# accre/lstore

Hardware: AMD Instinct MI355X
Metric: erasure encode+decode GiB/s (device-resident), RS(6+3) 1 MiB stripes (higher is better)
Workload: dtype u8; 1 GPU; reed_sol_van(6+3) encode + decode(lost shard 0), C=1048576 B per shard, 4096 stripes/GPU, k*C=6291456 B user data per stripe; method=reed_sol_van, k=6, m=3, chunk_bytes=1048576, packet_size=4096, stripes_per_gpu=4096, parallelism=static stripe partition x1

## Files before the change

### lstore_amd/csrc/ec_kernels.h

```cpp
#pragma once

#include <hip/hip_runtime.h>
#include <stdint.h>

#include <tuple>
#include <utility>

namespace lsec {

template <typename T, size_t... I>
hipError_t launch_packed(const void *k, dim3 grid, dim3 block, hipStream_t st, T &args, std::index_sequence<I...>) {
  void *ptrs[] = {static_cast<void *>(&std::get<I>(args))..., nullptr};
  return hipLaunchKernel(k, grid, block, ptrs, 0, st);
}
template <typename... KArgs, typename... Args>
hipError_t launch_kernel(void (*k)(KArgs...), dim3 grid, dim3 block, hipStream_t st, const Args &...args) {
  static_assert(sizeof...(KArgs) == sizeof...(Args), "argument count");
  std::tuple<std::decay_t<KArgs>...> t(static_cast<std::decay_t<KArgs>>(args)...);
  return launch_packed(reinterpret_cast<const void *>(k), grid, block, st, t, std::index_sequence_for<KArgs...>{});
}

size_t occupancy_lds_bytes(int64_t shard_bytes);
template <typename T, size_t... I>
hipError_t launch_packed_shm(const void *k, dim3 grid, dim3 block, size_t shm, hipStream_t st, T &args,
// ... 66 lines not shown
struct PatternArgs {
  const PatRecord *recs;
  const CoefCell *cells;
  const uint8_t *stripe_pattern;
  uint32_t npat;
  uint32_t rot0, rot_step, rot_n;
  int K;
  int nstripes;
  int packet;
  int nshards;
  int64_t size;
  unsigned *tiles;
  uint32_t tiles_pre;
  uint32_t tile_phase;
  ShardRef sh[kPatMaxShards];
};

hipError_t launch_pattern_bytewise(const PatternArgs &a, int rmax, hipStream_t stream);
hipError_t launch_pattern_bitsliced(const PatternArgs &a, int rmax, hipStream_t stream);

struct CheckArgs {
  const CoefCell *cells;
  int K, R;
  int nstripes;
  int packet;
  int64_t size;
  unsigned *syndrome;
  unsigned *bad_count;
  unsigned *tiles;
  uint32_t tiles_pre;
  uint32_t tile_phase;
  ShardRef in[kMaxK];
  ShardRef par[kMaxR];
};

hipError_t launch_check_bytewise(const CheckArgs &a, hipStream_t stream);
hipError_t launch_check_bitsliced(const CheckArgs &a, hipStream_t stream, int dw_pref = 0);

struct LocateArgs : CheckArgs {
  const CoefCell *ratio;
  unsigned long long *hyp;
};

constexpr unsigned kLocateClean = 0xFF, kLocateMany = 0xFE;

hipError_t launch_locate_bytewise(const LocateArgs &a, hipStream_t stream);
hipError_t launch_locate_bitsliced(const LocateArgs &a, hipStream_t stream, int dw_pref = 0);
hipError_t launch_locate_finalize(const unsigned *syndrome, unsigned long long *hyp, unsigned char *located,
                                  unsigned *counts, int nstripes, int K, int R, hipStream_t stream);

constexpr int kRotMaxShards = kMaxK + 8;
struct CheckRotArgs {
  const CoefCell *cells;
  int K, R;
  int nstripes;
  int packet;
  int64_t size;
  unsigned *syndrome;
  unsigned *bad_count;
  unsigned *tiles;
  uint32_t tiles_pre;
  uint32_t tile_phase;
  uint32_t rot0, rot_step, rot_n;
  ShardRef sh[kRotMaxShards];
};

struct LocateRotArgs : CheckRotArgs {
  const CoefCell *ratio;
  unsigned long long *hyp;
};

hipError_t launch_check_rot_bytewise(const CheckRotArgs &a, hipStream_t stream);
hipError_t launch_check_rot_bitsliced(const CheckRotArgs &a, hipStream_t stream, int dw_pref = 0);
hipError_t launch_locate_rot_bytewise(const LocateRotArgs &a, hipStream_t stream);
hipError_t launch_locate_rot_bitsliced(const LocateRotArgs &a, hipStream_t stream, int dw_pref = 0);
hipError_t launch_locate_finalize_rot(const unsigned *syndrome, unsigned long long *hyp, unsigned char *located,
                                      unsigned char *located_dev, unsigned *counts, unsigned *dev_faults, int nstripes,
                                      int K, int R, uint32_t rot0, uint32_t rot_step, uint32_t rot_n, hipStream_t stream);

struct PatternRotArgs : PatternArgs {};
hipError_t launch_pattern_rot_bytewise(const PatternRotArgs &a, hipStream_t stream);
hipError_t launch_pattern_rot_bitsliced(const PatternRotArgs &a, hipStream_t stream);

enum LaunchFamily { kFormChk = 1, kFormLoc, kFormChkRot, kFormLocRot, kFormPat, kFormPatRot };
struct LaunchForm {
  int family, sliced, R, KC, IT, VW, BF, DW;
};
constexpr int kLaunchRecordMax = 16;
void record_launch(const LaunchForm &f);
void launch_record_reset();
int launch_record(LaunchForm *out, int max);
bool predict_launch(int family, bool sliced, int K, int R, int packet, int dw_pref, LaunchForm *out);
int fixed_k_list(int *out, int max);

constexpr int kTileQueueLine = 32;
constexpr int kTileQueueWords = 9 * kTileQueueLine;
constexpr int kTileQueueRing = 4096;
constexpr uint64_t kTileQueueMinTiles = 16384;
unsigned *tile_queue_slot(hipStream_t st, uint64_t ntiles);
bool tile_phase_on();
bool tile_phase_net_on();
void set_tile_phase(int mode);
void tile_queue_release(hipStream_t st, unsigned *slot);
uint32_t tiles_prefix(uint32_t ntiles);
unsigned long long *launch_stamps(uint32_t *n);
void set_launch_stamps(unsigned long long *p, uint32_t n);
int persistent_grid(const void *kernel, int grid, hipStream_t st);

constexpr int kMaxMagicShards = kMaxK + kMaxR;

struct MagicArgs {
  int nshards;
  int shard0;
  int total_shards;
  int nstripes;
  int64_t size;
  int64_t col0;
  int64_t chunk;
  unsigned long long *acc;
  ShardRef sh[kMaxMagicShards];
};

hipError_t launch_stripe_magic(const MagicArgs &a, hipStream_t stream);
hipError_t launch_magic_finalize(const unsigned long long *acc, int nstripes, int64_t total_len, uint8_t *magic,
                                 hipStream_t stream);

struct DiffArgs {
  int npairs;
  int nstripes;
  int64_t size;
  int *flags;
  ShardRef a[kMaxR];
  ShardRef b[kMaxR];
};
hipError_t launch_chunk_diff(const DiffArgs &a, hipStream_t stream);

struct GatherPiece {
  uint64_t src;
  uint64_t dst_off;
  uint64_t bytes;
};
hipError_t launch_gather(const GatherPiece *list, int n, char *dst, hipStream_t stream);

constexpr uint32_t kPieceBytes = 16384;
struct CopyPiece {
  uint64_t src;
  uint64_t dst;
  uint64_t bytes;
};
hipError_t launch_copy_pieces(const CopyPiece *list, int n, hipStream_t stream);

hipError_t launch_signal(unsigned *counter, unsigned *flag, unsigned value, hipStream_t stream);

hipError_t launch_hbm_copy(void *dst, const void *src, uint64_t bytes, hipStream_t stream);
hipError_t launch_hbm_mix(const ApplyArgs &a, hipStream_t stream);
hipError_t launch_probe_xor(const ShardRef *in, int K, ShardRef out, int nstripes, int64_t size, int variant,
                            hipStream_t stream);

void make_cell(uint8_t c, CoefCell &cell);

hipError_t launch_bytewise(const ApplyArgs &a, hipStream_t stream, int grid_blocks = 0);
hipError_t launch_bytewise_magic(const ApplyArgs &a, hipStream_t stream, int grid_blocks = 0);
hipError_t launch_bitsliced(const ApplyArgs &a, hipStream_t stream, int grid_blocks = 0, int dw_pref = 0);
hipError_t launch_bitmatrix(const ApplyArgs &a, hipStream_t stream, int grid_blocks = 0);
bool bitmatrix_w_supported(int w);
hipError_t launch_wordwise(const ApplyArgs &a, hipStream_t stream, int grid_blocks = 0);
hipError_t launch_gfw_bitsliced(const ApplyArgs &a, hipStream_t stream, int grid_blocks = 0);
void make_word_cell(uint32_t c, int w, uint32_t *out);

void set_kernel_variant(int bytewise_variant, int bitsliced_variant);
void set_tile_mode(int mode);
int tile_mode();
int bytewise_variant();
int bitsliced_variant();

}
```

### lstore_amd/csrc/ec_kernels.hip

```cpp
#include <atomic>
#include <cstdio>
#include <cstdlib>
#include <cstring>
#include <map>
#include <mutex>
#include <type_traits>

#include "ec_hiperr.h"
#include "ec_kernels_impl.h"

namespace lsec {

namespace {

int g_bw_variant = 0, g_bs_variant = 0;

int default_grid(uint64_t ntiles) {
  return static_cast<int>(std::min<uint64_t>(std::max<uint64_t>(ntiles, 1), (1ull << 31) - 1));
}

constexpr int kQueueDevs = 64;
std::once_flag g_queue_once[kQueueDevs];
unsigned *g_queue[kQueueDevs];
std::atomic<uint32_t> g_queue_next[kQueueDevs];
// ... 152 lines not shown
int tile_phase_mode() {
  int v = g_tile_phase.load(std::memory_order_relaxed);
  if (v < 0) {
    const char *e = getenv("LSEC_TILE_PHASE");
    v = e && *e ? (atoi(e) & 3) : 1;
    int expect = -1;
    if (!g_tile_phase.compare_exchange_strong(expect, v)) v = expect;
  }
  return v;
}
}

bool tile_phase_on() { return (tile_phase_mode() & 1) != 0; }
bool tile_phase_net_on() { return (tile_phase_mode() & 2) != 0; }

void set_tile_phase(int mode) { g_tile_phase.store(mode & 3, std::memory_order_relaxed); }

size_t occupancy_lds_bytes(int64_t shard_bytes) {
  static const int cap = [] {
    const char *e = getenv("LSEC_WGS_CAP");
    return e ? std::max(0, atoi(e)) : 0;
  }();
  static const int64_t min_bytes = [] {
    const char *e = getenv("LSEC_WGS_CAP_MIN_KB");
    return e ? static_cast<int64_t>(atoll(e)) << 10 : 0;
  }();
  if (cap <= 0 || shard_bytes < min_bytes) return 0;
  const size_t per = (160u << 10) / static_cast<size_t>(cap);
  return per > (2u << 10) ? (per - (2u << 10)) & ~static_cast<size_t>(255) : 0;
}

int persistent_grid(const void *kernel, int grid, hipStream_t st) {
  const int dev = stream_device(st);
  if (dev < 0 || dev >= kQueueDevs || g_cus[dev] <= 0) return 0;
  static std::mutex mu;
  static std::map<const void *, int> per_cu;
  int n = 0;
  {
    std::lock_guard<std::mutex> lk(mu);
    auto it = per_cu.find(kernel);
    if (it != per_cu.end()) {
      n = it->second;
    } else {
      if (quiet([&] { return hipOccupancyMaxActiveBlocksPerMultiprocessor(&n, kernel, kBlock, 0); }) != hipSuccess) n = 0;
      per_cu[kernel] = n;
    }
  }
  static const int force = [] {
    const char *e = getenv("LSEC_TILES_WGS");
    return e ? atoi(e) : 0;
  }();
  if (force > 0) n = force;
  static const int cap = [] {
    const char *e = getenv("LSEC_WGS_CAP");
    return e ? std::max(0, atoi(e)) : 0;
  }();
  if (cap > 0 && n > cap) n = cap;
  if (n <= 0) return 0;
  const int full = n * g_cus[dev];
  const int pg = std::max(8, std::min(grid, full) & ~7);
  static const bool trace = getenv("LSEC_TRACE") != nullptr;
  if (trace) fprintf(stderr, "[lsec tiles] kernel %p: %d workgroups per CU x %d CUs -> grid %d (of %d tiles)\n", kernel, n, g_cus[dev], pg, grid);
  return pg;
}

void set_tile_mode(int mode) { g_tiles_mode.store(std::max(0, std::min(2, mode)), std::memory_order_relaxed); }

int tile_mode() { return tiles_mode(); }

uint32_t tiles_prefix(uint32_t ntiles) {
  if (tiles_mode() != 2) return 0;
  const uint64_t per = (static_cast<uint64_t>(ntiles) + 7) / 8;
  return static_cast<uint32_t>(per * prefix_64ths() / 64);
}

void set_kernel_variant(int bw, int bs) {
  g_bw_variant = bw;
  g_bs_variant = bs;
}

int bytewise_variant() { return g_bw_variant; }
int bitsliced_variant() { return g_bs_variant; }

hipError_t launch_bytewise(const ApplyArgs &a, hipStream_t st, int grid_blocks) {
  if (a.K < 1 || a.K > kMaxK || a.R < 1 || a.R > 8 || a.size % 8 != 0) return hipErrorInvalidValue;
  if (a.nstripes <= 0 || a.size == 0) return hipSuccess;
  const int shape = a.accumulate ? 1 : bytewise_shape(a.K, a.R);
  const int grid = tile_grid(bw_shape(shape).tile_bytes(), a.size, a.nstripes, grid_blocks);
  if (!grid) return hipErrorInvalidValue;
  return by_r(a.R, [&](auto r) { return dispatch_bytewise<decltype(r)::value>(a, st, grid, shape); });
}

hipError_t launch_bytewise_magic(const ApplyArgs &a, hipStream_t st, int grid_blocks) {
  if (a.K < 1 || a.K > kMaxK || a.R < 1 || a.R > 8 || a.size % 8 != 0 || !a.magic_acc) return hipErrorInvalidValue;
  if (a.nstripes <= 0 || a.size == 0) return hipSuccess;
  const int grid = tile_grid(BwShape{bytewise_magic_it(a.K), 4, true}.tile_bytes(), a.size, a.nstripes, grid_blocks);
  if (!grid) return hipErrorInvalidValue;
  return by_r(a.R, [&](auto r) { return dispatch_bytewise_magic<decltype(r)::value>(a, st, grid); });
}

hipError_t launch_bitsliced(const ApplyArgs &a, hipStream_t st, int grid_blocks, int dw_pref) {
  if (a.K < 1 || a.K > kMaxK || a.R < 1 || a.R > 8 || a.packet <= 0 || a.packet % 4 != 0 ||
      a.size % (8LL * a.packet) != 0)
    return hipErrorInvalidValue;
  if (a.nstripes <= 0 || a.size == 0) return hipSuccess;
  const int want = g_bs_variant != 0 ? g_bs_variant : dw_pref;
  const int dw = lane_dwords(!a.magic_acc && !a.accumulate ? want : 1, a.packet);
  const int grid = tile_grid(kBlock * 4ull * dw, a.size / 8, a.nstripes, grid_blocks);
  if (!grid) return hipErrorInvalidValue;
  return by_r(a.R, [&](auto r) { return dispatch_bitsliced<decltype(r)::value>(a, st, grid, dw); });
}

bool bitmatrix_w_supported(int w) {
  switch (w) {
#define LSEC_BM_CASE(WW) case WW:
    LSEC_BITMATRIX_W(LSEC_BM_CASE)
#undef LSEC_BM_CASE
    return true;
    default:
      return false;
  }
}

hipError_t launch_bitmatrix(const ApplyArgs &a, hipStream_t st, int grid_blocks) {
  if (a.K < 1 || a.K > kMaxK || a.R < 1 || a.R > 2 || a.w < 2 || a.w > kMaxW || !a.masks ||
      a.packet <= 0 || a.packet % 4 != 0 || a.size % (static_cast<int64_t>(a.w) * a.packet) != 0)
    return hipErrorInvalidValue;
  if (a.nstripes <= 0 || a.size == 0) return hipSuccess;
  const int grid = tile_grid(kBlock * 4, a.size / a.w, a.nstripes, grid_blocks);
  if (!grid) return hipErrorInvalidValue;
  return by_r(a.R, [&](auto r) { return dispatch_bitmatrix<decltype(r)::value>(a, st, grid); });
}

hipError_t launch_wordwise(const ApplyArgs &a, hipStream_t st, int grid_blocks) {
  if (a.K < 1 || a.K > kMaxK || a.R < 1 || a.R > 8 || (a.w != 16 && a.w != 32) || !a.masks || a.size % 8 != 0)
    return hipErrorInvalidValue;
  if (a.nstripes <= 0 || a.size == 0) return hipSuccess;
  const bool transposed = g_bs_variant != 10 && (a.w == 16 || a.R <= 4);
  const int grid = tile_grid(kBlock * (transposed ? 4ull * a.w : a.w == 16 ? 16ull : 8ull), a.size, a.nstripes, grid_blocks);
  if (!grid) return hipErrorInvalidValue;
  if (transposed) return by_r(a.R, [&](auto r) { return dispatch_gfw_transposed<decltype(r)::value>(a, st, grid); });
  return by_r(a.R, [&](auto r) { return dispatch_wordwise<decltype(r)::value>(a, st, grid); });
}

hipError_t launch_gfw_bitsliced(const ApplyArgs &a, hipStream_t st, int grid_blocks) {
  if (a.K < 1 || a.K > kMaxK || a.R < 1 || a.R > (a.w == 32 ? 4 : 8) || (a.w != 16 && a.w != 32) || !a.masks ||
      a.packet <= 0 || a.packet % 4 != 0 || a.size % (static_cast<int64_t>(a.w) * a.packet) != 0)
    return hipErrorInvalidValue;
  if (a.nstripes <= 0 || a.size == 0) return hipSuccess;
  const int grid = tile_grid(kBlock * 4, a.size / a.w, a.nstripes, grid_blocks);
  if (!grid) return hipErrorInvalidValue;
  return by_r(a.R, [&](auto r) { return dispatch_gfw_bitsliced<decltype(r)::value>(a, st, grid); });
}

namespace {
bool pattern_args_ok(const PatternArgs &a, int rmax) {
  return a.K >= 1 && a.K <= kMaxK && rmax >= 1 && rmax <= kPatMaxOut && a.recs && a.cells && a.npat >= 1 &&
         a.npat <= kPatMaxPatterns && a.nshards >= 1 && a.nshards <= kPatMaxShards && a.size % 8 == 0 &&
         (a.stripe_pattern || (a.rot_n >= 1 && a.rot0 < a.rot_n && a.rot_step < a.rot_n && a.rot_n <= a.npat));
}
}

hipError_t launch_pattern_bytewise(const PatternArgs &a, int rmax, hipStream_t st) {
  if (!pattern_args_ok(a, rmax)) return hipErrorInvalidValue;
  if (a.nstripes <= 0 || a.size == 0) return hipSuccess;
  const int grid = tile_grid(bw_auto(a.K, rmax).tile_bytes(), a.size, a.nstripes);
  if (!grid) return hipErrorInvalidValue;
  return by_r(rmax, [&](auto r) { return dispatch_pat_bytewise<decltype(r)::value>(a, st, grid); });
}
// ... 581 lines not shown
```

### lstore_amd/csrc/ec_kernels_impl.h

```cpp
#pragma once
#include "ec_kernels.h"

#include <algorithm>
#include <type_traits>

namespace lsec {

typedef uint32_t u32x2 __attribute__((ext_vector_type(2)));
typedef uint32_t u32x4 __attribute__((ext_vector_type(4)));

template <int N> struct VecT;
template <> struct VecT<1> { typedef uint32_t type; };
template <> struct VecT<2> { typedef u32x2 type; };
template <> struct VecT<4> { typedef u32x4 type; };

constexpr int kBlock = 256;

typedef const __attribute__((address_space(4))) CoefCell ConstCell;

__device__ __forceinline__ ConstCell *const_cells(const CoefCell *p) {
  return reinterpret_cast<ConstCell *>(reinterpret_cast<uintptr_t>(p));
}

#define LSEC_GLOBAL __attribute__((address_space(1)))
// ... 966 lines not shown
          put<ACC, u32x2>(q0 + o, h);
        }
      }
    }
  }
}

template <int R, int W, bool ACC = false>
__global__ __launch_bounds__(kBlock) void k_gfw_transposed(ApplyArgs a) {
  constexpr uint32_t kCoefMask = W == 16 ? 0xFFFFu : 0xFFFFFFFFu;
  ConstU32 *prod = reinterpret_cast<ConstU32 *>(reinterpret_cast<uintptr_t>(a.masks));
  bool xor_only = true;
  for (int i = 0; i < R * a.K && xor_only; ++i) xor_only = (prod[i * W] & kCoefMask) <= 1u;
  if (xor_only)
    gfw_transposed_tiles<R, W, true, ACC>(a);
  else
    gfw_transposed_tiles<R, W, false, ACC>(a);
}

#define LSEC_BITMATRIX_W(X) X(2) X(3) X(4) X(5) X(6) X(7) X(8) X(10) X(11) X(12) X(13) X(16) X(17) \
                            X(18) X(19) X(22) X(23) X(28) X(29) X(30) X(31) X(32)

#define LSEC_FIXED_K(X) X(4) X(6) X(8) X(10) X(12) X(16) X(20)
constexpr bool has_fixed_k(int K) {
#define LSEC_IS_K(KK) \
  if (K == KK) return true;
  LSEC_FIXED_K(LSEC_IS_K)
#undef LSEC_IS_K
  return false;
}

struct BwShape {
  int it, vw;
  bool bf;
  constexpr uint64_t tile_bytes() const { return static_cast<uint64_t>(kBlock) * 4 * vw * it; }
};
constexpr int kBwShapes = 5;
constexpr BwShape bw_shape(int code) {
  return code == 0 ? BwShape{2, 4, true} : code == 1 ? BwShape{1, 4, true} : code == 2 ? BwShape{2, 2, true}
       : code == 3 ? BwShape{1, 2, true} : BwShape{1, 2, false};
}
constexpr int bw_auto_code(int K, int R) { return R == 1 ? 4 : K >= 16 ? 1 : 0; }
constexpr BwShape bw_auto(int K, int R) { return bw_shape(bw_auto_code(K, R)); }
constexpr int bytewise_magic_it(int K) { return bw_auto(K, 2).it; }

template <int R, int IT, bool BF, int VW>
hipError_t bytewise_k(const ApplyArgs &a, hipStream_t st, int grid) {
  switch (a.K) {
#define LSEC_BW_K(KK) \
  case KK: return launch_tiled(&k_gf8_bytewise<R, KK, IT, BF, VW>, grid, st, a);
    LSEC_FIXED_K(LSEC_BW_K)
#undef LSEC_BW_K
    default: return launch_tiled(&k_gf8_bytewise<R, 0, IT, BF, VW>, grid, st, a);
  }
}

template <int R>
hipError_t dispatch_bytewise(const ApplyArgs &a, hipStream_t st, int grid, int shape) {
  if (a.accumulate) {
    return launch_tiled(&k_gf8_bytewise<R, 0, 1, true, 4, false, true>, grid, st, a);
  }
  switch (shape) {
    case 1: return bytewise_k<R, 1, true, 4>(a, st, grid);
    case 2: return bytewise_k<R, 2, true, 2>(a, st, grid);
    case 3: return bytewise_k<R, 1, true, 2>(a, st, grid);
    case 4: return bytewise_k<R, 1, false, 2>(a, st, grid);
    default: return bytewise_k<R, 2, true, 4>(a, st, grid);
  }
}

template <int R>
hipError_t dispatch_bytewise_magic(const ApplyArgs &a, hipStream_t st, int grid) {
  switch (a.K) {
#define LSEC_BWM_K(KK) \
  case KK: return launch_tiled(&k_gf8_bytewise<R, KK, bytewise_magic_it(KK), true, 4, true>, grid, st, a);
    LSEC_FIXED_K(LSEC_BWM_K)
#undef LSEC_BWM_K
    default:
      if (bytewise_magic_it(a.K) == 1) return launch_tiled(&k_gf8_bytewise<R, 0, 1, true, 4, true>, grid, st, a);
      return launch_tiled(&k_gf8_bytewise<R, 0, 2, true, 4, true>, grid, st, a);
  }
}

template <int R>
hipError_t dispatch_bitsliced(const ApplyArgs &a, hipStream_t st, int grid, int dw) {
  if (a.magic_acc) {
    return launch_tiled(&k_gf8_bitsliced<R, 0, 1, true>, grid, st, a);
  }
  if (a.accumulate) {
    return launch_tiled(&k_gf8_bitsliced<R, 0, 1, false, true>, grid, st, a);
  }
  switch (dw) {
    case 4: return launch_tiled(&k_gf8_bitsliced<R, 0, 4>, grid, st, a);
    case 2: return launch_tiled(&k_gf8_bitsliced<R, 0, 2>, grid, st, a);
    default: return launch_tiled(&k_gf8_bitsliced<R, 0, 1>, grid, st, a);
  }
}

template <int R>
hipError_t dispatch_bitmatrix(const ApplyArgs &a, hipStream_t st, int grid) {
  if constexpr (R <= 2) {
    if (a.accumulate) {
      return launch_kernel(&k_bitmatrix_any<R>, dim3(grid), dim3(kBlock), st, a);
    }
    switch (a.w) {
#define LSEC_BM_W(WW) \
  case WW: return launch_kernel(&k_bitmatrix<R, WW>, dim3(grid), dim3(kBlock), st, a);
      LSEC_BITMATRIX_W(LSEC_BM_W)
#undef LSEC_BM_W
      default: return launch_kernel(&k_bitmatrix_any<R>, dim3(grid), dim3(kBlock), st, a);
    }
  } else {
    return hipErrorInvalidValue;
  }
}

template <int R>
hipError_t dispatch_wordwise(const ApplyArgs &a, hipStream_t st, int grid) {
  switch (a.w * 2 + (a.accumulate ? 1 : 0)) {
    case 32: return launch_kernel(&k_gfw_wordwise<R, 16>, dim3(grid), dim3(kBlock), st, a);
    case 33: return launch_kernel(&k_gfw_wordwise<R, 16, true>, dim3(grid), dim3(kBlock), st, a);
    case 64: return launch_kernel(&k_gfw_wordwise<R, 32>, dim3(grid), dim3(kBlock), st, a);
    case 65: return launch_kernel(&k_gfw_wordwise<R, 32, true>, dim3(grid), dim3(kBlock), st, a);
    default: return hipErrorInvalidValue;
  }
}

template <int R>
hipError_t dispatch_gfw_transposed(const ApplyArgs &a, hipStream_t st, int grid) {
  if (a.w == 16) {
    if (a.accumulate) return launch_kernel(&k_gfw_transposed<R, 16, true>, dim3(grid), dim3(kBlock), st, a);
    else return launch_kernel(&k_gfw_transposed<R, 16>, dim3(grid), dim3(kBlock), st, a);
  } else if constexpr (R <= 4) {
    if (a.w != 32) return hipErrorInvalidValue;
    if (a.accumulate) return launch_kernel(&k_gfw_transposed<R, 32, true>, dim3(grid), dim3(kBlock), st, a);
    else return launch_kernel(&k_gfw_transposed<R, 32>, dim3(grid), dim3(kBlock), st, a);
  } else {
    return hipErrorInvalidValue;
  }
}

template <int R>
hipError_t dispatch_gfw_bitsliced(const ApplyArgs &a, hipStream_t st, int grid) {
  if (a.w == 16) {
    if (a.accumulate) return launch_kernel(&k_gfw_bitsliced<R, 16, true>, dim3(grid), dim3(kBlock), st, a);
    else return launch_kernel(&k_gfw_bitsliced<R, 16>, dim3(grid), dim3(kBlock), st, a);
  } else if constexpr (R <= 4) {
    if (a.w != 32) return hipErrorInvalidValue;
    if (a.accumulate) return launch_kernel(&k_gfw_bitsliced<R, 32, true>, dim3(grid), dim3(kBlock), st, a);
    else return launch_kernel(&k_gfw_bitsliced<R, 32>, dim3(grid), dim3(kBlock), st, a);
  } else {
    return hipErrorInvalidValue;
  }
}

typedef const __attribute__((address_space(4))) PatRecord ConstRec;

__device__ __forceinline__ uint32_t stripe_pattern_id(const PatternArgs &a, uint32_t s) {
  if (a.stripe_pattern)
    return __builtin_amdgcn_readfirstlane(static_cast<uint32_t>(*gptr<uint8_t>(reinterpret_cast<uint64_t>(a.stripe_pattern) + s)));
  return (a.rot0 + (s % a.rot_n) * a.rot_step) % a.rot_n;
}

template <typename Args>
__device__ __forceinline__ uint32_t rot_back(const Args &a, uint32_t s) {
  return __builtin_amdgcn_readfirstlane(a.rot_n - (a.rot0 + (s % a.rot_n) * a.rot_step) % a.rot_n);
// ... 761 lines not shown
```

### lstore_amd/csrc/ec_plan.cpp

```cpp
#include <hip/hip_runtime.h>

#include <algorithm>
#include <atomic>
#include <chrono>
#include <cstdarg>
#include <cstring>
#include <map>
#include <memory>
#include <mutex>
#include <string>
#include <thread>
#include <vector>

#include <strings.h>

#include <array>
#include <cstdio>

#include "ec_jit.h"
#include "ec_engine.h"

#include <unistd.h>

extern "C" const char *JE_method[N_JE_METHODS] = {"reed_sol_van", "reed_sol_r6_op", "cauchy_orig", "cauchy_good",
// ... 1603 lines not shown
  const void *cells = nullptr;
  if (decode_entry(e, ids, &ent, &cells)) return -1;
  (void)lsec::jit::wait(cells, 30000);
  return 0;
}

int lsec_prepare_encode(lio_erasure_plan_t *plan) {
  PlanExt *e = ext_of(plan);
  if (!e) return fail("not an lstore_ec plan");
  const void *cells = nullptr;
  if (encode_cells(e, &cells)) return -1;
  (void)lsec::jit::wait(cells, 30000);
  return 0;
}

int lsec_plan_jit(lio_erasure_plan_t *plan, const int *erasures) {
  PlanExt *e = ext_of(plan);
  if (!e) return 0;
  const int kind = kernel_kind(e->pub.method, e->pub.w);
  if (kind == KBYTEWISE ? lsec::bytewise_variant() != 0
                        : (kind == KWORDWISE || kind == KBITMATRIX || kind == KBITSLICEDW || kind == KBITSLICED)
                            ? lsec::bitsliced_variant() != 0
                            : true)
    return 0;
  const void *cells = nullptr;
  int R = 0;
  if (!erasures) {
    if (encode_cells(e, &cells)) return 0;
    R = encode_rows(e);
  } else {
    std::vector<int> ids;
    DecodeEntry *ent = nullptr;
    if (parse_erasures(plan, erasures, ids) != 0 || decode_entry(e, ids, &ent, &cells)) return 0;
    R = static_cast<int>(ent->dp.erased.size());
  }
  if (kind == KBITSLICED && plan->w == 8 && cauchy8_bitsliced_dw(plan->data_strips, R, plan->strip_size) > 0) return 0;
  return lsec::jit::ready(cells, R, plan->data_strips) != nullptr ? 1 : 0;
}

int lsec_plan_kernel(lio_erasure_plan_t *plan) { return plan ? kernel_kind(plan->method, plan->w) : 0; }

void lsec_set_kernel_variant(int bytewise_variant, int bitsliced_variant) {
  lsec::set_kernel_variant(bytewise_variant, bitsliced_variant);
}

void lsec_set_tile_sharing(int mode) { lsec::set_tile_mode(mode); }

int lsec_tile_sharing(void) { return lsec::tile_mode(); }

void lsec_test_set_stamps(void *dev_buf, unsigned n) {
  lsec::set_launch_stamps(static_cast<unsigned long long *>(dev_buf), n);
}

int lsec_test_apply_path(void) { return tl_apply_path; }

int lsec_test_launch_record(int *forms, int max_forms) {
  lsec::LaunchForm rec[lsec::kLaunchRecordMax];
  const int n = lsec::launch_record(rec, lsec::kLaunchRecordMax);
  for (int i = 0; forms && i < n && i < max_forms && i < lsec::kLaunchRecordMax; ++i) {
    const int v[8] = {rec[i].family, rec[i].sliced, rec[i].R, rec[i].KC, rec[i].IT, rec[i].VW, rec[i].BF, rec[i].DW};
    std::memcpy(forms + 8 * i, v, sizeof(v));
  }
  return n;
}

int lsec_test_predict_form(int family, int plan_kernel, int K, int R, int packet, long long block_size, int *form) {
  if (!form) return fail("lsec_test_predict_form: NULL output");
  if (plan_kernel != KBYTEWISE && plan_kernel != KBITSLICED) return fail("lsec_test_predict_form: plan kernel %d", plan_kernel);
  const bool sliced = plan_kernel == KBITSLICED;
  lsec::LaunchForm f;
  if (!lsec::predict_launch(family, sliced, K, R, packet, sliced ? cauchy8_bitsliced_dw(K, R, block_size) : 0, &f))
    return fail("lsec_test_predict_form: no kernel of family %d for K=%d R=%d packet=%d", family, K, R, packet);
  const int v[8] = {f.family, f.sliced, f.R, f.KC, f.IT, f.VW, f.BF, f.DW};
  std::memcpy(form, v, sizeof(v));
  return 0;
}

int lsec_test_fixed_k(int *out, int max) { return lsec::fixed_k_list(out, max); }

void lsec_test_set_cauchy8_policy(int mode) { g_c8_policy.store(mode == 1 ? 1 : 0, std::memory_order_relaxed); }

void lsec_test_set_tile_phase(int mode) { lsec::set_tile_phase(mode); }

void lsec_test_set_pattern_split(int stripes) { g_pattern_split.store(std::max(0, stripes), std::memory_order_relaxed); }

int lsec_test_pattern_table(lio_erasure_plan_t *plan, const int *patterns, int npatterns, const int *lost, int n_shift,
                            int pattern_id, int *nout, int *in_sel, int *out_sel, int *coef) {
  PlanExt *e = ext_of(plan);
  if (!e) return fail("not an lstore_ec plan");
  if (!nout || !in_sel || !out_sel || !coef) return fail("lsec_test_pattern_table: NULL output");
  PatternTable tab;
  if (build_pattern_table(e, patterns, npatterns, lost, n_shift, tab)) return -1;
  if (pattern_id < 0 || pattern_id >= static_cast<int>(tab.recs.size()))
    return fail("lsec_test_pattern_table: entry %d outside 0..%zu", pattern_id, tab.recs.size() - 1);
  const lsec::PatRecord &rec = tab.recs[pattern_id];
  const int k = plan->data_strips;
  *nout = tab.reachable[pattern_id] ? static_cast<int>(rec.nout) : -1;
  for (int j = 0; j < k; ++j) in_sel[j] = rec.nout ? static_cast<int>(rec.in_sel[j]) : -1;
  for (uint32_t r = 0; r < rec.nout; ++r) {
    out_sel[r] = static_cast<int>(rec.out_sel[r]);
    for (int j = 0; j < k; ++j) coef[r * k + j] = static_cast<int>(tab.cells[rec.cells_off + r * k + j].coef);
  }
  for (int r = static_cast<int>(rec.nout); rec.nout && r < tab.rmax; ++r)
    for (int j = 0; j < k; ++j)
      if (tab.cells[rec.cells_off + static_cast<size_t>(r) * k + j].coef != 0 ||
          tab.cells[rec.cells_off + static_cast<size_t>(r) * k + j].ta_lo != 0)
        return fail("lsec_test_pattern_table: entry %d row %d is not zero", pattern_id, r);
  return 0;
}

int lsec_test_locate_ratio(lio_erasure_plan_t *plan, int r, int j) {
  PlanExt *e = ext_of(plan);
  if (!e) return fail("not an lstore_ec plan");
  const int kind = kernel_kind(plan->method, plan->w);
  if (kind != KBYTEWISE && kind != KBITSLICED) return fail("lsec_test_locate_ratio: plan kernel %d", kind);
  if (plan->parity_strips < 2) return fail("lsec_test_locate_ratio: m=%d", plan->parity_strips);
  const lsec::gf8::Mat *q = nullptr;
  if (locate_ratio(e, &q)) return -1;
  if (r < 0 || r >= plan->parity_strips - 1 || j < 0 || j >= plan->data_strips)
    return fail("lsec_test_locate_ratio: [%d][%d] outside %d x %d", r, j, plan->parity_strips - 1, plan->data_strips);
  return (*q)[static_cast<size_t>(r) * plan->data_strips + j];
}

int lsec_test_pattern_rot0(int n, int n_shift, long long first_stripe) {
  if (n < 1 || n_shift < 0 || first_stripe < 0) return fail("lsec_test_pattern_rot0: n >= 1, n_shift >= 0, first_stripe >= 0");
  return static_cast<int>(pattern_rot0(n, n_shift, first_stripe));
}


int lsec_selftest_bit_decode(int method, int k, int w) {
  std::vector<int> bm = method == LIBERATION   ? lsec::gf8::liberation_bitmatrix(k, w)
                        : method == BLAUM_ROTH ? lsec::gf8::blaum_roth_bitmatrix(k, w)
                        : method == LIBER8TION ? lsec::gf8::liber8tion_bitmatrix(k)
                                               : std::vector<int>();
  if (bm.empty()) return fail("lsec_selftest_bit_decode: no %d bitmatrix for k=%d w=%d", method, k, w);
  const int m = 2;
  int n = 0;
  for (int a = 0; a < k + m; ++a)
    for (int b = a; b < k + m; ++b) {
      std::vector<int> ids = a == b ? std::vector<int>{a} : std::vector<int>{a, b};
      lsec::gf8::DecodePlan p1, p2;
      std::vector<uint32_t> m1, m2;
      const bool ok1 = lsec::gf8::make_bit_decode(k, m, w, bm, ids, p1, m1);
      const bool ok2 = lsec::gf8::make_bit_decode_dense(k, m, w, bm, ids, p2, m2);
      if (ok1 != ok2 || p1.survivors != p2.survivors || p1.erased != p2.erased || m1 != m2)
        return fail("lsec_selftest_bit_decode: erasures {%d, %d} differ (ok %d/%d)", a, b, ok1, ok2);
      ++n;
    }
  return n;
}

}
```

### lstore_amd/erasure.py

```python
from __future__ import annotations

import collections
import ctypes as C
import os
import subprocess
from typing import Iterable, Sequence

import numpy as np

HERE = os.path.dirname(os.path.abspath(__file__))
ROOT = os.path.dirname(HERE)
_LIB_PATH = os.path.join(HERE, "liblstore_ec.so")

REED_SOL_VAN, REED_SOL_R6_OP, CAUCHY_ORIG, CAUCHY_GOOD, BLAUM_ROTH, LIBERATION, LIBER8TION, RAID4 = range(8)
JE_METHOD_NAMES = ("reed_sol_van", "reed_sol_r6_op", "cauchy_orig", "cauchy_good", "blaum_roth",
                   "liberation", "liber8tion", "raid4")


class ErasureError(RuntimeError):
    pass


class PlanStruct(C.Structure):
    """src/lio/erasure_tools.h:50-65"""
# ... 28 lines not shown
class ShardRef(C.Structure):
    _fields_ = [("base", C.c_void_p), ("stride", C.c_longlong)]


EXPORTS = ("nearest_prime", "et_method_type", "et_new_plan", "et_generate_plan", "et_destroy_plan",
           "et_encode", "et_decode", "et_encode_stripes", "et_decode_stripes", "lsec_encode_dev",
           "lsec_decode_dev", "et_encode_stripes_magic", "et_stripes_magic", "lsec_encode_magic_dev",
           "lsec_stripe_magic_dev", "lsec_segment_write", "lsec_segment_write_iov", "lsec_segment_encode_iov",
           "lsec_segment_straddle_bytes", "lsec_segment_read", "lsec_segment_inspect",
           "lsec_prepare_decode", "lsec_abi_version", "lsec_device_count", "lsec_last_error", "lsec_plan_kernel",
           "lsec_set_kernel_variant", "lsec_set_host_devices", "lsec_hbm_copy_dev", "lsec_hbm_mix_dev", "lsec_prepare_encode", "lsec_plan_jit", "lsec_device_numa",
           "lsec_set_tile_sharing", "lsec_tile_sharing", "lsec_host_unpin_drain", "lsec_hbm_decode_shape_dev",
           "lsec_decode_dev_patterns", "lsec_decode_dev_rotated", "lsec_check_dev", "lsec_locate_dev",
           "lsec_check_dev_rotated", "lsec_locate_dev_rotated")

READ_PARANOID, MAGIC_LEGACY, INSPECT_FIX, MAX_DEVS = 1, 2, 4, 256
LOCATE_CLEAN, LOCATE_MANY, LOCATE_REPAIR = 0xFF, 0xFE, 1
STRIPE_OK, STRIPE_EMPTY, STRIPE_BAD_MAGIC, STRIPE_REPAIRED, STRIPE_LOST_MAGIC, STRIPE_LOST_MISMATCH = range(6)


class InspectState(C.Structure):
    _fields_ = [("bad_stripes", C.c_longlong), ("unrecoverable", C.c_longlong), ("silent_errors", C.c_longlong),
                ("empty_stripes", C.c_longlong), ("brute_used", C.c_int),
                ("brute_badmap", C.c_ubyte * MAX_DEVS)]

_lib = None


def library_path() -> str:
    return _LIB_PATH


def build_library(force: bool = False) -> str:
    if force or not os.path.exists(_LIB_PATH):
        jobs = str(min(8, os.cpu_count() or 1))
        subprocess.run(["make", "-s", "-j", jobs, "-C", os.path.join(HERE, "csrc")], check=True)
    return _LIB_PATH


def lib():
    global _lib
    if _lib is not None:
        return _lib
    if not os.path.exists(_LIB_PATH):
        raise ErasureError(f"{_LIB_PATH} is not built; run lstore_amd.build_library() "
                           "(or `make -C lstore_amd/csrc`)")
    L = C.CDLL(_LIB_PATH)
    P = C.POINTER(PlanStruct)
    L.et_generate_plan.restype = P
    L.et_generate_plan.argtypes = [C.c_longlong, C.c_int, C.c_int, C.c_int, C.c_int, C.c_int, C.c_int]
    L.et_new_plan.restype = P
    L.et_new_plan.argtypes = [C.c_int, C.c_longlong, C.c_int, C.c_int, C.c_int, C.c_int, C.c_int]
    L.et_destroy_plan.argtypes = [P]
    L.et_destroy_plan.restype = None
    L.et_method_type.argtypes = [C.c_char_p]
    L.nearest_prime.argtypes = [C.c_int, C.c_int]
    L.et_encode.argtypes = [P, C.c_char_p, C.c_longlong, C.c_char_p, C.c_longlong, C.c_int]
    L.et_decode.argtypes = [P, C.c_longlong, C.c_char_p, C.c_longlong, C.c_char_p, C.c_longlong, C.c_int,
                            C.POINTER(C.c_int)]
    L.et_encode_stripes.argtypes = [P, C.POINTER(C.c_void_p), C.c_int, C.c_int]
    L.et_decode_stripes.argtypes = [P, C.POINTER(C.c_void_p), C.c_int, C.c_int, C.POINTER(C.c_int)]
    L.lsec_encode_dev.argtypes = [P, C.POINTER(ShardRef), C.c_int, C.c_longlong, C.c_void_p]
    L.lsec_decode_dev.argtypes = [P, C.POINTER(ShardRef), C.c_int, C.c_longlong, C.POINTER(C.c_int), C.c_void_p]
    L.lsec_decode_dev_patterns.argtypes = [P, C.POINTER(ShardRef), C.c_int, C.c_longlong, C.POINTER(C.c_int), C.c_int,
                                           C.c_void_p, C.c_void_p]
    L.lsec_decode_dev_rotated.argtypes = [P, C.POINTER(ShardRef), C.c_int, C.c_longlong, C.POINTER(C.c_int), C.c_int,
                                          C.c_longlong, C.c_void_p]
    L.lsec_check_dev.argtypes = [P, C.POINTER(ShardRef), C.c_int, C.c_longlong, C.c_void_p, C.c_void_p, C.c_void_p]
    L.lsec_locate_dev.argtypes = [P, C.POINTER(ShardRef), C.c_int, C.c_longlong, C.c_void_p, C.c_void_p, C.c_void_p,
                                  C.c_void_p, C.c_int, C.c_void_p]
    L.lsec_check_dev_rotated.argtypes = [P, C.POINTER(ShardRef), C.c_int, C.c_longlong, C.c_int, C.c_longlong, C.c_void_p,
                                         C.c_void_p, C.c_void_p]
    L.lsec_locate_dev_rotated.argtypes = [P, C.POINTER(ShardRef), C.c_int, C.c_longlong, C.c_int, C.c_longlong, C.c_void_p,
                                          C.c_void_p, C.c_void_p, C.c_void_p, C.c_void_p, C.c_void_p, C.c_int, C.c_void_p]
    L.lsec_test_locate_ratio.argtypes = [P, C.c_int, C.c_int]
    L.lsec_test_set_pattern_split.argtypes = [C.c_int]
    L.lsec_test_set_pattern_split.restype = None
    L.lsec_test_pattern_table.argtypes = [P, C.POINTER(C.c_int), C.c_int, C.POINTER(C.c_int), C.c_int, C.c_int,
                                          C.POINTER(C.c_int), C.POINTER(C.c_int), C.POINTER(C.c_int), C.POINTER(C.c_int)]
    L.lsec_test_pattern_rot0.argtypes = [C.c_int, C.c_int, C.c_longlong]
    L.lsec_test_launch_record.argtypes = [C.POINTER(C.c_int), C.c_int]
    L.lsec_test_predict_form.argtypes = [C.c_int, C.c_int, C.c_int, C.c_int, C.c_int, C.c_longlong, C.POINTER(C.c_int)]
    L.lsec_test_fixed_k.argtypes = [C.POINTER(C.c_int), C.c_int]
    L.lsec_prepare_decode.argtypes = [P, C.POINTER(C.c_int)]
    L.lsec_prepare_encode.argtypes = [P]
    L.lsec_plan_jit.argtypes = [P, C.POINTER(C.c_int)]
    L.et_encode_stripes_magic.argtypes = [P, C.POINTER(C.c_void_p), C.c_int, C.c_int, C.c_void_p]
    L.et_stripes_magic.argtypes = [P, C.POINTER(C.c_void_p), C.c_int, C.c_int, C.c_void_p]
    L.lsec_encode_magic_dev.argtypes = [P, C.POINTER(ShardRef), C.c_int, C.c_longlong, C.c_void_p, C.c_void_p]
    L.lsec_stripe_magic_dev.argtypes = [P, C.POINTER(ShardRef), C.c_int, C.c_longlong, C.c_void_p, C.c_void_p]
    L.lsec_segment_write.argtypes = [P, C.c_void_p, C.c_int, C.c_int, C.c_int, C.c_longlong, C.c_void_p]
    L.lsec_segment_write_iov.argtypes = [P, C.c_void_p, C.c_int, C.c_int, C.c_int, C.c_int, C.c_longlong, C.c_void_p]
    L.lsec_segment_encode_iov.argtypes = [P, C.c_void_p, C.c_int, C.c_int, C.c_int, C.c_void_p, C.c_void_p, C.c_void_p,
                                          C.c_longlong, C.c_void_p, C.c_int]
    L.lsec_segment_straddle_bytes.restype = C.c_longlong
    L.lsec_segment_straddle_bytes.argtypes = [P, C.c_void_p, C.c_int, C.c_int, C.c_int]
    L.lsec_segment_read.argtypes = [P, C.c_void_p, C.c_int, C.c_int, C.c_int, C.c_longlong, C.c_int, C.c_void_p,
                                    C.c_void_p]
    L.lsec_segment_inspect.argtypes = [P, C.c_void_p, C.c_int, C.c_int, C.c_int, C.c_void_p, C.c_void_p, C.c_void_p,
                                       C.POINTER(InspectState)]
    L.lsec_last_error.restype = C.c_char_p
    L.lsec_plan_kernel.argtypes = [P]
    L.lsec_set_kernel_variant.argtypes = [C.c_int, C.c_int]
    L.lsec_set_kernel_variant.restype = None
    L.lsec_set_tile_sharing.argtypes = [C.c_int]
    L.lsec_set_tile_sharing.restype = None
    L.lsec_tile_sharing.restype = C.c_int
    L.lsec_host_unpin_drain.argtypes = []
    L.lsec_host_unpin_drain.restype = C.c_int
    L.lsec_set_host_devices.argtypes = [C.POINTER(C.c_int), C.c_int]
    L.lsec_hbm_copy_dev.argtypes = [C.c_void_p, C.c_void_p, C.c_ulonglong, C.c_void_p]
    L.lsec_hbm_mix_dev.argtypes = [C.c_void_p, C.c_int, C.c_int, C.c_int, C.c_longlong, C.c_void_p]
    L.lsec_hbm_decode_shape_dev.argtypes = [C.c_void_p, C.c_int, C.c_int, C.c_longlong, C.c_int, C.c_void_p]
    L.lsec_device_numa.argtypes = [C.c_int, C.POINTER(C.c_int), C.POINTER(C.c_int), C.c_int]
    L.lsec_test_numa_for_bus.argtypes = [C.c_char_p, C.c_char_p, C.POINTER(C.c_int), C.POINTER(C.c_int), C.c_int]
    L.lsec_test_server_hold.restype = C.c_longlong
    L.lsec_test_server_hold.argtypes = [C.c_int, C.c_int]
    _lib = L
    return L


def last_error() -> str:
    return (lib().lsec_last_error() or b"").decode()


def _check(rc: int, what: str) -> int:
    if rc != 0:
        raise ErasureError(f"{what} failed (rc={rc}): {last_error()}")
    return rc


def _erasure_array(erasures: Iterable[int]):
    vals = list(erasures) + [-1]
    return (C.c_int * len(vals))(*vals)


def _pattern_array(patterns):
    vals = []
    for pat in patterns:
        vals += [int(x) for x in pat] + [-1]
    return (C.c_int * max(1, len(vals)))(*vals)


def nearest_prime(w: int, which: int) -> int:
    return lib().nearest_prime(w, which)


def method_type(name: str) -> int:
    return lib().et_method_type(name.encode())


class Plan:

    def __init__(self, ptr):
        if not ptr:
            raise ErasureError(f"plan creation failed: {last_error()}")
        self._p = ptr

    @classmethod
    def generate(cls, file_size, method, k, m, w=-1, packet_low=-1, packet_high=-1) -> "Plan":
        return cls(lib().et_generate_plan(file_size, method, k, m, w, packet_low, packet_high))

    @classmethod
    def new(cls, method, strip_size, k, m, w, packet_size, base_unit=8) -> "Plan":
        return cls(lib().et_new_plan(method, strip_size, k, m, w, packet_size, base_unit))

# ... 311 lines not shown
    def check_dev_rotated_refs(self, refs, nstripes: int, block_size: int, n_shift: int, first_stripe: int,
                               syndrome_ptr: int, bad_count_ptr: int = 0, stream: int = 0) -> None:
        _check(lib().lsec_check_dev_rotated(self._p, None if refs is None else self.shard_refs(refs), nstripes, block_size,
                                            n_shift, first_stripe, syndrome_ptr or None, bad_count_ptr or None, stream),
               "lsec_check_dev_rotated")

    def locate_dev_rotated_refs(self, refs, nstripes: int, block_size: int, n_shift: int, first_stripe: int,
                                syndrome_ptr: int, hyp_ptr: int, located_ptr: int, located_dev_ptr: int = 0,
                                counts_ptr: int = 0, dev_faults_ptr: int = 0, repair: bool = False, stream: int = 0) -> None:
        _check(lib().lsec_locate_dev_rotated(self._p, None if refs is None else self.shard_refs(refs), nstripes, block_size,
                                             n_shift, first_stripe, syndrome_ptr or None, hyp_ptr or None,
                                             located_ptr or None, located_dev_ptr or None, counts_ptr or None,
                                             dev_faults_ptr or None, LOCATE_REPAIR if repair else 0, stream),
               "lsec_locate_dev_rotated")

    def prepare_decode(self, erasures) -> None:
        _check(lib().lsec_prepare_decode(self._p, _erasure_array(erasures)), "lsec_prepare_decode")

    def prepare_encode(self) -> None:
        _check(lib().lsec_prepare_encode(self._p), "lsec_prepare_encode")

    def jit(self, erasures=None) -> bool:
        return bool(lib().lsec_plan_jit(self._p, None if erasures is None else _erasure_array(erasures)))


def _stream_handle(stream) -> int:
    if stream is None:
        import torch
        return torch.cuda.current_stream().cuda_stream
    if isinstance(stream, int):
        return stream
    return stream.cuda_stream


def device_count() -> int:
    return lib().lsec_device_count()


def set_host_devices(devices: Sequence[int] = ()) -> None:
    arr = (C.c_int * max(1, len(devices)))(*devices)
    _check(lib().lsec_set_host_devices(arr, len(devices)), "lsec_set_host_devices")


def device_numa(dev: int) -> tuple[int, list[int]]:
    node = C.c_int(-1)
    cpus = (C.c_int * 4096)()
    n = lib().lsec_device_numa(dev, C.byref(node), cpus, 4096)
    if n < 0:
        raise ErasureError(f"lsec_device_numa failed: {last_error()}")
    return node.value, list(cpus[:n])


def numa_for_bus(root: str, bus: str) -> tuple[int, list[int]]:
    node = C.c_int(-1)
    cpus = (C.c_int * 4096)()
    n = lib().lsec_test_numa_for_bus(root.encode(), bus.encode(), C.byref(node), cpus, 4096)
    if n < 0:
        raise ErasureError(f"lsec_test_numa_for_bus failed: {last_error()}")
    return node.value, list(cpus[:n])


TILES_STATIC, TILES_SHARED, TILES_TAIL = 0, 1, 2


def set_tile_sharing(mode) -> None:
    lib().lsec_set_tile_sharing(int(mode))


def tile_sharing() -> int:
    return int(lib().lsec_tile_sharing())


def set_kernel_variant(bytewise: int = 0, bitsliced: int = 0) -> None:
    lib().lsec_set_kernel_variant(bytewise, bitsliced)


PATH_NETWORK, PATH_PACKET_NETWORK, PATH_GENERIC = 1, 2, 4


def apply_path() -> int:
    return int(lib().lsec_test_apply_path())


FORM_FAMILIES = ("chk", "loc", "chkrot", "locrot", "pat", "patrot")
Form = collections.namedtuple("Form", "family sliced R KC IT VW BF DW")
Form.__doc__ = """One separately compiled kernel of the check / locate / patterned / rotated calls: family (one of
FORM_FAMILIES), sliced (plan kernel 2), R rows; bytewise: KC (0 = K at run time), IT steps of VW dwords
per lane, BF branch-free; bit-sliced: DW dwords per lane (the others 0)."""


def _form(v) -> Form:
    return Form(FORM_FAMILIES[v[0] - 1], bool(v[1]), *(int(x) for x in v[2:8]))


def launch_record() -> list:
    buf = (C.c_int * (8 * 16))()
    n = lib().lsec_test_launch_record(buf, 16)
    if n > 16:
        raise ErasureError(f"lsec_test_launch_record: {n} launches, 16 are kept")
    return [_form(buf[8 * i:8 * i + 8]) for i in range(n)]


def predict_form(family: str, plan_kernel: int, k: int, rows: int, packet: int = 0, block_size: int = 0) -> Form:
    out = (C.c_int * 8)()
    _check(lib().lsec_test_predict_form(FORM_FAMILIES.index(family) + 1, plan_kernel, k, rows, packet, block_size, out),
           "lsec_test_predict_form")
    return _form(out)


def predict_forms(call: str, plan_kernel: int, k: int, rows: int, packet: int = 0, block_size: int = 0,
                  repair: bool = False) -> list:
    forms = [predict_form(call, plan_kernel, k, rows, packet, block_size)]
    if repair:
        forms.append(predict_form({"loc": "pat", "locrot": "patrot"}[call], plan_kernel, k, 1, packet, block_size))
    return forms


def fixed_k() -> tuple:
    buf = (C.c_int * 64)()
    return tuple(buf[:lib().lsec_test_fixed_k(buf, 64)])


def set_pattern_split(stripes: int = 0) -> None:
    lib().lsec_test_set_pattern_split(int(stripes))


def pattern_rot0(n: int, n_shift: int, first_stripe: int) -> int:
    return _check_nonneg(lib().lsec_test_pattern_rot0(n, n_shift, first_stripe), "lsec_test_pattern_rot0")


def _check_nonneg(rc: int, what: str) -> int:
    if rc < 0:
        raise ErasureError(f"{what} failed (rc={rc}): {last_error()}")
    return rc


def pattern_table_entry(plan: "Plan", pattern_id: int, patterns=None, lost=None, n_shift: int = 0):
    k, n = plan.k, plan.k + plan.m
    nout = C.c_int(0)
    in_sel, out_sel, coef = (C.c_int * k)(), (C.c_int * n)(), (C.c_int * (n * k))()
    pats = None if patterns is None else list(patterns)
    _check(lib().lsec_test_pattern_table(plan.ptr, None if pats is None else _pattern_array(pats),
                                         0 if pats is None else len(pats),
                                         None if lost is None else _erasure_array(lost), n_shift, pattern_id,
                                         C.byref(nout), in_sel, out_sel, coef), "lsec_test_pattern_table")
    e = max(0, nout.value)
    return nout.value, list(in_sel[:k]), list(out_sel[:e]), np.array(coef[:e * k], dtype=np.int32).reshape(e, k)


def host_unpin_drain() -> None:
    lib().lsec_host_unpin_drain()


def locate_ratio(plan: "Plan", r: int, j: int) -> int:
    return _check_nonneg(lib().lsec_test_locate_ratio(plan.ptr, r, j), "lsec_test_locate_ratio")
```

Before: 2188 GiB/s.

## Add burst-timed grouped-store kernel for single-output bytewise decode

```diff
diff --git a/lstore_amd/csrc/ec_burst_inst.hip b/lstore_amd/csrc/ec_burst_inst.hip
--- /dev/null
+++ b/lstore_amd/csrc/ec_burst_inst.hip
@@ -0,0 +1,2 @@
+#define LSEC_INSTANTIATING_BURST 1
+#include "ec_kernels_impl.h"
diff --git a/lstore_amd/csrc/ec_kernels.h b/lstore_amd/csrc/ec_kernels.h
--- a/lstore_amd/csrc/ec_kernels.h
+++ b/lstore_amd/csrc/ec_kernels.h
@@ -172,7 +172,8 @@
 hipError_t launch_pattern_rot_bytewise(const PatternRotArgs &a, hipStream_t stream);
 hipError_t launch_pattern_rot_bitsliced(const PatternRotArgs &a, hipStream_t stream);
 
-enum LaunchFamily { kFormChk = 1, kFormLoc, kFormChkRot, kFormLocRot, kFormPat, kFormPatRot };
+enum LaunchFamily { kFormChk = 1, kFormLoc, kFormChkRot, kFormLocRot, kFormPat, kFormPatRot,
+                    kFormDecBurst };
 struct LaunchForm {
   int family, sliced, R, KC, IT, VW, BF, DW;
 };
@@ -251,6 +252,19 @@
 
 hipError_t launch_bytewise(const ApplyArgs &a, hipStream_t stream, int grid_blocks = 0);
 hipError_t launch_bytewise_magic(const ApplyArgs &a, hipStream_t stream, int grid_blocks = 0);
+
+struct BurstArgs : ApplyArgs {
+  uint32_t burst_period;
+  uint32_t burst_window;
+};
+constexpr int kBurstTile = 2048;
+constexpr int kBurstDefault = 8;
+constexpr uint32_t kBurstPeriod = 2400;
+constexpr uint32_t kBurstWindow = 300;
+constexpr int64_t kBurstMinChunk = 512 << 10, kBurstMaxChunk = 1 << 20;
+constexpr uint64_t kBurstMinTiles = 1u << 18;
+void set_decode_burst(int g, int period, int window, int force);
+int decode_burst_choice(int K, int R, int64_t size, int nstripes, int accumulate, int *kc);
 hipError_t launch_bitsliced(const ApplyArgs &a, hipStream_t stream, int grid_blocks = 0, int dw_pref = 0);
 hipError_t launch_bitmatrix(const ApplyArgs &a, hipStream_t stream, int grid_blocks = 0);
 bool bitmatrix_w_supported(int w);
diff --git a/lstore_amd/csrc/ec_kernels.hip b/lstore_amd/csrc/ec_kernels.hip
--- a/lstore_amd/csrc/ec_kernels.hip
+++ b/lstore_amd/csrc/ec_kernels.hip
@@ -258,9 +258,64 @@
 int bytewise_variant() { return g_bw_variant; }
 int bitsliced_variant() { return g_bs_variant; }
 
+namespace {
+struct BurstSetting {
+  int g, force;
+  uint32_t period, window;
+};
+std::mutex g_burst_mu;
+BurstSetting g_burst{-1, 0, 0, 0};
+
+BurstSetting burst_setting() {
+  std::lock_guard<std::mutex> lk(g_burst_mu);
+  if (g_burst.g < 0) {
+    const char *e = getenv("LSEC_DECODE_BURST"), *p = getenv("LSEC_DECODE_BURST_PERIOD"), *w = getenv("LSEC_DECODE_BURST_WINDOW");
+    const int g = e && *e ? atoi(e) : kBurstDefault;
+    g_burst.g = g == 4 || g == 8 ? g : 0;
+    g_burst.force = 0;
+    g_burst.period = p && *p ? static_cast<uint32_t>(std::max(0, atoi(p))) : kBurstPeriod;
+    g_burst.window = w && *w ? static_cast<uint32_t>(std::max(0, atoi(w))) : kBurstWindow;
+  }
+  return g_burst;
+}
+}
+
+void set_decode_burst(int g, int period, int window, int force) {
+  std::lock_guard<std::mutex> lk(g_burst_mu);
+  if (g < 0) {
+    g_burst.g = -1;
+    return;
+  }
+  g_burst = BurstSetting{g == 4 || g == 8 ? g : 0, force ? 1 : 0, static_cast<uint32_t>(std::max(0, period)),
+                         static_cast<uint32_t>(std::max(0, window))};
+}
+
+int decode_burst_choice(int K, int R, int64_t size, int nstripes, int accumulate, int *kc) {
+  if (kc) *kc = 0;
+  if (K < 1 || K > kMaxK || R != 1 || accumulate || nstripes <= 0 || size <= 0 || size % 8 != 0) return 0;
+  if (bytewise_shape(K, R) != bw_auto_code(K, 1)) return 0;
+  const BurstSetting b = burst_setting();
+  if (b.g == 0 || size / kBurstTile < b.g) return 0;
+  const uint64_t ntiles = static_cast<uint64_t>((size + kBurstTile - 1) / kBurstTile) * static_cast<uint64_t>(nstripes);
+  if (!b.force && (ntiles < kBurstMinTiles || size < kBurstMinChunk || size > kBurstMaxChunk || !burst_fixed_k(K))) return 0;
+  if (kc) *kc = burst_fixed_k(K);
+  return b.g;
+}
+
 hipError_t launch_bytewise(const ApplyArgs &a, hipStream_t st, int grid_blocks) {
   if (a.K < 1 || a.K > kMaxK || a.R < 1 || a.R > 8 || a.size % 8 != 0) return hipErrorInvalidValue;
   if (a.nstripes <= 0 || a.size == 0) return hipSuccess;
+  if (const int G = grid_blocks > 0 ? 0 : decode_burst_choice(a.K, a.R, a.size, a.nstripes, a.accumulate, nullptr)) {
+    BurstArgs b;
+    static_cast<ApplyArgs &>(b) = a;
+    const BurstSetting set = burst_setting();
+    b.burst_period = set.period;
+    b.burst_window = set.window;
+    const uint64_t tps = static_cast<uint64_t>((a.size + kBurstTile - 1) / kBurstTile), gps = static_cast<uint64_t>(a.size / kBurstTile) / G;
+    const uint64_t units = (gps + (tps > gps * G ? 1 : 0)) * static_cast<uint64_t>(a.nstripes);
+    if (tps * static_cast<uint64_t>(a.nstripes) >= (1ull << 31)) return hipErrorInvalidValue;
+    return dispatch_decode_burst(b, st, default_grid(units), G);
+  }
   const int shape = a.accumulate ? 1 : bytewise_shape(a.K, a.R);
   const int grid = tile_grid(bw_shape(shape).tile_bytes(), a.size, a.nstripes, grid_blocks);
   if (!grid) return hipErrorInvalidValue;
diff --git a/lstore_amd/csrc/ec_kernels_impl.h b/lstore_amd/csrc/ec_kernels_impl.h
--- a/lstore_amd/csrc/ec_kernels_impl.h
+++ b/lstore_amd/csrc/ec_kernels_impl.h
@@ -1072,6 +1072,105 @@
   }
 }
 
+hipError_t dispatch_decode_burst(const BurstArgs &a, hipStream_t st, int grid, int G);
+#define LSEC_BURST_K(X) X(6) X(8) X(10) X(12) X(16)
+constexpr int burst_fixed_k(int K) {
+#define LSEC_IS_K(KK) \
+  if (K == KK) return KK;
+  LSEC_BURST_K(LSEC_IS_K)
+#undef LSEC_IS_K
+  return 0;
+}
+#ifdef LSEC_INSTANTIATING_BURST
+constexpr int kBurstMaxSleeps = 2048;
+
+template <int KC, int G>
+__global__ __launch_bounds__(kBlock) __attribute__((amdgpu_waves_per_eu(8, 8))) void k_gf8_decode_burst(BurstArgs a) {
+  typedef u32x2 V;
+  constexpr int kTile = BwTile<1, 2>::kBytes, kLane = 8;
+  static_assert(kTile == kBurstTile, "the R = 1 automatic shape's tile");
+  const int K = KC ? KC : a.K;
+  const int64_t C = a.size;
+  const uint32_t tps = static_cast<uint32_t>((C + kTile - 1) / kTile);
+  const uint32_t gps = static_cast<uint32_t>(C / kTile) / G;
+  const uint32_t ups = gps + (tps > gps * G ? 1u : 0u);
+  const uint32_t nunits = ups * static_cast<uint32_t>(a.nstripes);
+  ConstCell *cells = const_cells(a.cells);
+
+  const auto whole_tile = [&](uint32_t s, uint32_t t) LSEC_INLINE -> V {
+    V acc[1][1];
+    acc[0][0] = 0u;
+    const int64_t off = static_cast<int64_t>(t) * kTile + threadIdx.x * kLane;
+    bw_inputs<1, KC, 1, 2, false, false>(
+        acc, cells, K, [&](int j) LSEC_INLINE -> uint64_t { return a.in[j].base + s * a.in[j].stride + off; }, NoLoads());
+    return acc[0][0];
+  };
+
+  for_tiles<1>(nunits, a.tiles, a.tiles_pre, [&](uint32_t u) {
+    const uint32_t s = u / ups, i = u - s * ups;
+    const uint64_t q = a.out[0].base + s * a.out[0].stride;
+    if (i < gps) {
+      const uint32_t t0 = i * G;
+      V r[G];
+#pragma unroll
+      for (int g = 0; g < G; ++g) r[g] = whole_tile(s, t0 + g);
+#pragma unroll
+      for (int g = 0; g < G; ++g) asm volatile("" : "+v"(r[g]));
+      if (a.burst_period) {
+        const uint32_t c0 = static_cast<uint32_t>(__builtin_amdgcn_s_memrealtime());
+        const uint32_t ph = c0 % a.burst_period;
+        if (ph >= a.burst_window) {
+          const uint32_t need = a.burst_period - ph;
+          for (int n = 0; n < kBurstMaxSleeps; ++n) {
+            __builtin_amdgcn_s_sleep(2);
+            if (static_cast<uint32_t>(__builtin_amdgcn_s_memrealtime()) - c0 >= need) break;
+          }
+        }
+      }
+      const uint64_t q0 = q + static_cast<uint64_t>(t0) * kTile + threadIdx.x * kLane;
+#pragma unroll
+      for (int g = 0; g < G; ++g) put_nt<false, V>(q0 + static_cast<uint64_t>(g) * kTile, r[g]);
+    } else {
+      for (uint32_t t = gps * G; t < tps; ++t) {
+        const int64_t o = static_cast<int64_t>(t) * kTile + threadIdx.x * kLane;
+        if (static_cast<int64_t>(t + 1) * kTile <= C) {
+          put_nt<false, V>(q + o, whole_tile(s, t));
+        } else {
+          V acc[1][1];
+          acc[0][0] = 0u;
+          for (int j = 0; j < K; ++j) {
+            V v[1];
+            v[0] = load_ragged<2>(a.in[j].base + s * a.in[j].stride, o, C);
+            bw_accumulate<1, 1, 2>(acc, v, cells, K, j);
+          }
+          store_ragged<false, 2>(q, o, C, acc[0][0]);
+        }
+      }
+    }
+  }, a.tile_phase);
+}
+
+template <int KC>
+hipError_t decode_burst_k(const BurstArgs &a, hipStream_t st, int grid, int G) {
+  record_launch({kFormDecBurst, 0, 1, KC, 1, 2, 0, G});
+  switch (G) {
+    case 4: return launch_tiled(&k_gf8_decode_burst<KC, 4>, grid, st, a);
+    case 8: return launch_tiled(&k_gf8_decode_burst<KC, 8>, grid, st, a);
+    default: return hipErrorInvalidValue;
+  }
+}
+
+hipError_t dispatch_decode_burst(const BurstArgs &a, hipStream_t st, int grid, int G) {
+  switch (burst_fixed_k(a.K)) {
+#define LSEC_BURST_CASE(KK) \
+  case KK: return decode_burst_k<KK>(a, st, grid, G);
+    LSEC_BURST_K(LSEC_BURST_CASE)
+#undef LSEC_BURST_CASE
+    default: return decode_burst_k<0>(a, st, grid, G);
+  }
+}
+#endif
+
 template <int R>
 hipError_t dispatch_bitsliced(const ApplyArgs &a, hipStream_t st, int grid, int dw) {
   if (a.magic_acc) {
diff --git a/lstore_amd/csrc/ec_plan.cpp b/lstore_amd/csrc/ec_plan.cpp
--- a/lstore_amd/csrc/ec_plan.cpp
+++ b/lstore_amd/csrc/ec_plan.cpp
@@ -1709,6 +1709,16 @@
 
 void lsec_test_set_tile_phase(int mode) { lsec::set_tile_phase(mode); }
 
+void lsec_test_set_decode_burst(int g, int period, int window, int force) { lsec::set_decode_burst(g, period, window, force); }
+
+void lsec_test_launch_record_reset(void) { lsec::launch_record_reset(); }
+
+int lsec_test_decode_burst_choice(int K, int R, long long block_size, int nstripes, int accumulate, int *form) {
+  if (!form) return fail("lsec_test_decode_burst_choice: NULL output");
+  form[0] = lsec::decode_burst_choice(K, R, block_size, nstripes, accumulate, &form[1]);
+  return 0;
+}
+
 void lsec_test_set_pattern_split(int stripes) { g_pattern_split.store(std::max(0, stripes), std::memory_order_relaxed); }
 
 int lsec_test_pattern_table(lio_erasure_plan_t *plan, const int *patterns, int npatterns, const int *lost, int n_shift,
diff --git a/lstore_amd/erasure.py b/lstore_amd/erasure.py
--- a/lstore_amd/erasure.py
+++ b/lstore_amd/erasure.py
@@ -134,6 +134,11 @@
     L.lsec_test_launch_record.argtypes = [C.POINTER(C.c_int), C.c_int]
     L.lsec_test_predict_form.argtypes = [C.c_int, C.c_int, C.c_int, C.c_int, C.c_int, C.c_longlong, C.POINTER(C.c_int)]
     L.lsec_test_fixed_k.argtypes = [C.POINTER(C.c_int), C.c_int]
+    L.lsec_test_set_decode_burst.argtypes = [C.c_int, C.c_int, C.c_int, C.c_int]
+    L.lsec_test_set_decode_burst.restype = None
+    L.lsec_test_launch_record_reset.argtypes = []
+    L.lsec_test_launch_record_reset.restype = None
+    L.lsec_test_decode_burst_choice.argtypes = [C.c_int, C.c_int, C.c_longlong, C.c_int, C.c_int, C.POINTER(C.c_int)]
     L.lsec_prepare_decode.argtypes = [P, C.POINTER(C.c_int)]
     L.lsec_prepare_encode.argtypes = [P]
     L.lsec_plan_jit.argtypes = [P, C.POINTER(C.c_int)]
@@ -611,11 +616,12 @@
     return int(lib().lsec_test_apply_path())
 
 
-FORM_FAMILIES = ("chk", "loc", "chkrot", "locrot", "pat", "patrot")
+FORM_FAMILIES = ("chk", "loc", "chkrot", "locrot", "pat", "patrot", "decburst")
 Form = collections.namedtuple("Form", "family sliced R KC IT VW BF DW")
 Form.__doc__ = """One separately compiled kernel of the check / locate / patterned / rotated calls: family (one of
 FORM_FAMILIES), sliced (plan kernel 2), R rows; bytewise: KC (0 = K at run time), IT steps of VW dwords
-per lane, BF branch-free; bit-sliced: DW dwords per lane (the others 0)."""
+per lane, BF branch-free; bit-sliced: DW dwords per lane (the others 0).  decburst (the burst form of the
+single-output decode, appended by decode_dev): DW holds its tiles per group."""
 
 
 def _form(v) -> Form:
@@ -630,6 +636,10 @@
     return [_form(buf[8 * i:8 * i + 8]) for i in range(n)]
 
 
+def launch_record_reset() -> None:
+    lib().lsec_test_launch_record_reset()
+
+
 def predict_form(family: str, plan_kernel: int, k: int, rows: int, packet: int = 0, block_size: int = 0) -> Form:
     out = (C.c_int * 8)()
     _check(lib().lsec_test_predict_form(FORM_FAMILIES.index(family) + 1, plan_kernel, k, rows, packet, block_size, out),
@@ -643,6 +653,17 @@
     if repair:
         forms.append(predict_form({"loc": "pat", "locrot": "patrot"}[call], plan_kernel, k, 1, packet, block_size))
     return forms
+
+
+def set_decode_burst(group: int, period: int = 2400, window: int = 300, force: bool = False) -> None:
+    lib().lsec_test_set_decode_burst(group, period, window, int(force))
+
+
+def decode_burst_choice(k: int, rows: int, block_size: int, nstripes: int, accumulate: bool = False) -> tuple:
+    out = (C.c_int * 2)()
+    _check(lib().lsec_test_decode_burst_choice(k, rows, block_size, nstripes, int(accumulate), out),
+           "lsec_test_decode_burst_choice")
+    return int(out[0]), int(out[1])
 
 
 def fixed_k() -> tuple:
```

Result: faster. 2232 GiB/s (median of 6 runs) (+2.0%).
